# autonomousvision/unimatch

Measured on NVIDIA H100. Metric: image-pairs/sec @480x832 gmflow-scale2-refine6; EPE vs reference, higher is better.
Workload: dtype fp32

## Files before the change

### unimatch_b200/csrc/um_attention_tc.cu

```cuda
#include <math_constants.h>

#include "um_common.cuh"
#include "um_tc.cuh"

namespace um {

using namespace tc;

namespace {

constexpr int BM = 128, BN = 64;
constexpr int NTHREADS = 288;
constexpr int PRODUCER = 8;
constexpr uint32_t Q_BYTES = 4 * 16384;
constexpr uint32_t KV_STAGE_BYTES = 4 * 8192;
constexpr uint32_t OFF_Q = 0;
constexpr uint32_t OFF_K = OFF_Q + Q_BYTES;
constexpr uint32_t OFF_V = OFF_K + 2 * KV_STAGE_BYTES;
constexpr uint32_t OFF_X = OFF_V + 2 * KV_STAGE_BYTES;
constexpr uint32_t OFF_BAR = OFF_X + 1024;
constexpr uint32_t OFF_KREG = OFF_BAR + 256;
constexpr int MAX_LP = 2048;
constexpr uint32_t SMEM_BYTES = OFF_KREG + MAX_LP;
constexpr float SQRT_C = 11.313708498984761f;
constexpr float EXP_SCALE = 1.4426950408889634f / 11.313708498984761f;
constexpr float LAZY_THRESH = 8.0f / EXP_SCALE;

struct TcParams {
  float* out; long long ldo;
  int n_streams, kv_shift, lp;
  Geom g;
  const float* values; int vdim, value_mode, post_op;
  float* dbg;
  __half* out_split; long long split_plane;
};

__device__ __forceinline__ uint32_t pack_h2(__half a, __half b) {
  return (uint32_t)__half_as_ushort(a) | ((uint32_t)__half_as_ushort(b) << 16);
}

template <bool HAS_V>
__global__ void __launch_bounds__(NTHREADS, 1)
attn_tc_kernel(const __grid_constant__ CUtensorMap map_q, const __grid_constant__ CUtensorMap map_k,
               const __grid_constant__ CUtensorMap map_v, TcParams p) {
  extern __shared__ __align__(1024) uint8_t smem[];
  uint64_t* bars = reinterpret_cast<uint64_t*>(smem + OFF_BAR);
  uint64_t* q_full = bars + 0;
  uint64_t* k_full = bars + 1;
  uint64_t* k_empty = bars + 3;
  uint64_t* v_full = bars + 5;
  uint64_t* v_empty = bars + 7;
  int8_t* kreg = reinterpret_cast<int8_t*>(smem + OFF_KREG);

  const Geom g = p.g;
  const int warp = threadIdx.x >> 5, lane = threadIdx.x & 31;
  const int m0 = blockIdx.x * BM, win = blockIdx.y, n = blockIdx.z;
  const int nk = (n + p.kv_shift) % p.n_streams;
  const int nwin = g.nwin, lp = p.lp;
  const int T = (g.lw + BN - 1) / BN;
  const int planes = p.n_streams * nwin * lp;

  if (threadIdx.x == 0) {
    mbar_init(q_full, 1);
    for (int i = 0; i < 2; ++i) {
      mbar_init(k_full + i, 1); mbar_init(k_empty + i, 8);
      mbar_init(v_full + i, 1); mbar_init(v_empty + i, 8);
    }
    fence_barrier_init();
  }
  if (warp == PRODUCER && lane == 0) { tma_prefetch_desc(&map_q); tma_prefetch_desc(&map_k); tma_prefetch_desc(&map_v); }
  bool masked = false;
  if (g.mask_mode == UM_MASK_SWIN) {
    const int wy = win / g.kw, wx = win - wy * g.kw;
    masked = (g.sh > 0 && wy == g.kh - 1) || (g.sw > 0 && wx == g.kw - 1);
    if (masked)
      for (int t = threadIdx.x; t < g.lw; t += NTHREADS) {
        int yr, xr;
        window_token(g, win, t, &yr, &xr);
        kreg[t] = (int8_t)shift_region(g, yr, xr);
      }
  }
  __syncthreads();

  if (warp == PRODUCER) {
    const int qrow = (n * nwin + win) * lp + m0;
    if (elect_one()) {
      mbar_arrive_expect_tx(q_full, Q_BYTES);
#pragma unroll
      for (int part = 0; part < 2; ++part)
#pragma unroll
        for (int half = 0; half < 2; ++half)
          tma_load_2d(smem + OFF_Q + (part * 2 + half) * 16384, &map_q, q_full, half * 64, part * planes + qrow);
    }
    __syncwarp();
    const int krow = (nk * nwin + win) * lp;
    auto load_tile = [&](int j, const CUtensorMap* map, uint32_t off, uint64_t* full, uint64_t* empty) {
      const int s = j & 1;
      mbar_wait_inline(empty + s, ((j >> 1) & 1) ^ 1);
      if (elect_one()) {
        mbar_arrive_expect_tx(full + s, KV_STAGE_BYTES);
#pragma unroll
        for (int part = 0; part < 2; ++part)
#pragma unroll
          for (int half = 0; half < 2; ++half)
            tma_load_2d(smem + off + s * KV_STAGE_BYTES + (part * 2 + half) * 8192, map, full + s, half * 64,
                        part * planes + krow + j * BN);
      }
      __syncwarp();
    };
    load_tile(0, &map_k, OFF_K, k_full, k_empty);
    for (int j = 0; j < T; ++j) {
      if (j + 1 < T) load_tile(j + 1, &map_k, OFF_K, k_full, k_empty);
      if (HAS_V) load_tile(j, &map_v, OFF_V, v_full, v_empty);
    }
    return;
  }

  const int cw = warp;
  const int wg = cw >> 2;
  const int fr = wg * 64 + (cw & 3) * 16 + (lane >> 2);
  const int fc = 2 * (lane & 3);
  int rq[2] = {0, 0}, tok[2];
  bool row_valid[2];
#pragma unroll
  for (int h = 0; h < 2; ++h) {
    const int tq = m0 + fr + 8 * h;
    row_valid[h] = tq < g.lw;
    int yr = 0, xr = 0;
    tok[h] = row_valid[h] ? window_token(g, win, tq, &yr, &xr) : -1;
    if (masked) rq[h] = shift_region(g, yr, xr);
  }
  float m_run[2] = {-CUDART_INF_F, -CUDART_INF_F}, l_run[2] = {0.f, 0.f};
  const uint32_t q_base = smem_u32(smem + OFF_Q) + wg * 8192;
  auto consumers_sync = [&]() { asm volatile("bar.sync 1, 256;" ::: "memory"); };

  auto compute_s = [&](int j, float (&sv)[32]) {
    const int s = j & 1;
    mbar_wait_inline(k_full + s, (j >> 1) & 1);
    const uint32_t k_base = smem_u32(smem + OFF_K + s * KV_STAGE_BYTES);
    const int qa[3] = {1, 0, 0}, kb[3] = {0, 1, 0};
    fence_acc(sv);
    wgmma_fence();
#pragma unroll
    for (int c = 0; c < 3; ++c)
#pragma unroll
      for (int half = 0; half < 2; ++half)
#pragma unroll
        for (int ks = 0; ks < 4; ++ks)
          wgmma_ss<BN>(sv, desc_kmajor(q_base + (qa[c] * 2 + half) * 16384 + ks * 32),
                       desc_kmajor(k_base + (kb[c] * 2 + half) * 8192 + ks * 32), (c | half | ks) != 0);
    wgmma_commit();
    wgmma_wait<0>();
    fence_acc(sv);
    __syncwarp();
    if (lane == 0) mbar_arrive(k_empty + s);
  };
  mbar_wait_inline(q_full, 0);

  if (!HAS_V) {
    float* vals = reinterpret_cast<float*>(smem + OFF_X);
    const int et = threadIdx.x;
    const long long L = (long long)g.h * g.w;
    float a0[2] = {0.f, 0.f}, a1[2] = {0.f, 0.f};
    for (int j = 0; j < T; ++j) {
      const int s = j & 1;
      const int n0 = j * BN;
      if (et < BN) {
        float v0 = 0.f, v1 = 0.f;
        const int t = n0 + et;
        if (t < g.lw) {
          const int ktok = window_token(g, win, t);
          if (p.value_mode == UM_VALUE_TENSOR) {
            const float* vp = p.values + ((long long)nk * L + ktok) * p.vdim;
            v0 = __ldg(vp); v1 = (p.vdim > 1) ? __ldg(vp + 1) : 0.f;
          } else {
            const int ky = ktok / g.w;
            v0 = (float)(ktok - ky * g.w); v1 = (float)ky;
          }
        }
        vals[(s * BN + et) * 2] = v0; vals[(s * BN + et) * 2 + 1] = v1;
      }
      float sv[32];
      compute_s(j, sv);
      consumers_sync();
      const float2* vv = reinterpret_cast<const float2*>(vals + s * BN * 2);
#pragma unroll
      for (int h = 0; h < 2; ++h) {
        float mx = -CUDART_INF_F;
#pragma unroll
        for (int jj = 0; jj < 8; ++jj)
#pragma unroll
          for (int e = 0; e < 2; ++e) {
            float& x = sv[4 * jj + 2 * h + e];
            if (n0 + 8 * jj + fc + e >= g.lw) x = -CUDART_INF_F;
            mx = fmaxf(mx, x);
          }
        mx = fmaxf(mx, __shfl_xor_sync(0xffffffffu, mx, 1));
        mx = fmaxf(mx, __shfl_xor_sync(0xffffffffu, mx, 2));
        const float m_new = fmaxf(m_run[h], mx);
        const float alpha = exp2f((m_run[h] - m_new) * EXP_SCALE);
        m_run[h] = m_new;
        const float mscaled = m_new * EXP_SCALE;
        float sum = 0.f, b0 = 0.f, b1 = 0.f;
#pragma unroll
        for (int jj = 0; jj < 8; ++jj)
#pragma unroll
          for (int e = 0; e < 2; ++e) {
            const float pe = ex2_approx(fmaf(sv[4 * jj + 2 * h + e], EXP_SCALE, -mscaled));
            const float2 kv = vv[8 * jj + fc + e];
            sum += pe;
            b0 = fmaf(pe, kv.x, b0);
            b1 = fmaf(pe, kv.y, b1);
          }
        l_run[h] = l_run[h] * alpha + sum;
        a0[h] = a0[h] * alpha + b0;
        a1[h] = a1[h] * alpha + b1;
      }
    }
#pragma unroll
    for (int h = 0; h < 2; ++h) {
#pragma unroll
      for (int o = 1; o <= 2; o <<= 1) {
        l_run[h] += __shfl_xor_sync(0xffffffffu, l_run[h], o);
        a0[h] += __shfl_xor_sync(0xffffffffu, a0[h], o);
        a1[h] += __shfl_xor_sync(0xffffffffu, a1[h], o);
      }
      if (row_valid[h] && (lane & 3) == 0) {
        float r0 = a0[h] / l_run[h], r1 = a1[h] / l_run[h];
        const int oy = tok[h] / g.w, ox = tok[h] - oy * g.w;
        if (p.post_op == UM_POST_MINUS_OWN) { r0 -= (float)ox; r1 -= (float)oy; }
        else if (p.post_op == UM_POST_OWN_MINUS) { r0 = (float)ox - r0; }
        float* dst = p.out + ((long long)n * L + tok[h]) * p.vdim;
        dst[0] = r0;
        if (p.vdim > 1) dst[1] = r1;
      }
    }
    return;
  }

  float o[64];
#pragma unroll
  for (int i = 0; i < 64; ++i) o[i] = 0.f;
  const bool dump = p.dbg && blockIdx.x == 0 && blockIdx.y == 0 && blockIdx.z == 0;
  for (int j = 0; j < T; ++j) {
    const int s = j & 1;
    const int n0 = j * BN;
    float sv[32];
    compute_s(j, sv);
    if (dump && j == 0)
#pragma unroll
      for (int i = 0; i < 32; ++i) p.dbg[(fr + 8 * ((i >> 1) & 1)) * BN + 8 * (i >> 2) + fc + (i & 1)] = sv[i];
    uint32_t ph[16], pl[16];
#pragma unroll
    for (int h = 0; h < 2; ++h) {
#pragma unroll
      for (int jj = 0; jj < 8; ++jj)
#pragma unroll
        for (int e = 0; e < 2; ++e) {
          const int col = n0 + 8 * jj + fc + e;
          float& x = sv[4 * jj + 2 * h + e];
          if (masked && kreg[col < g.lw ? col : 0] != rq[h]) x -= 100.0f * SQRT_C;
          if (col >= g.lw) x = -CUDART_INF_F;
        }
      float mx = -CUDART_INF_F;
#pragma unroll
      for (int jj = 0; jj < 8; ++jj) mx = fmaxf(mx, fmaxf(sv[4 * jj + 2 * h], sv[4 * jj + 2 * h + 1]));
      mx = fmaxf(mx, __shfl_xor_sync(0xffffffffu, mx, 1));
      mx = fmaxf(mx, __shfl_xor_sync(0xffffffffu, mx, 2));
      float alpha = 1.0f;
      if (mx > m_run[h] + LAZY_THRESH) {
        alpha = exp2f((m_run[h] - mx) * EXP_SCALE);
        m_run[h] = mx;
#pragma unroll
        for (int jj = 0; jj < 16; ++jj) { o[4 * jj + 2 * h] *= alpha; o[4 * jj + 2 * h + 1] *= alpha; }
      }
      const float mscaled = m_run[h] * EXP_SCALE;
      float sum = 0.f;
#pragma unroll
      for (int jj = 0; jj < 8; ++jj) {
        const float p0 = ex2_approx(fmaf(sv[4 * jj + 2 * h], EXP_SCALE, -mscaled));
        const float p1 = ex2_approx(fmaf(sv[4 * jj + 2 * h + 1], EXP_SCALE, -mscaled));
        sum += p0 + p1;
        split_f16x2(p0, p1, &ph[2 * jj + h], &pl[2 * jj + h]);
      }
      l_run[h] = l_run[h] * alpha + sum;
    }
    mbar_wait_inline(v_full + s, (j >> 1) & 1);
    const uint32_t v_base = smem_u32(smem + OFF_V + s * KV_STAGE_BYTES);
    fence_acc(o);
    wgmma_fence();
#pragma unroll
    for (int c = 0; c < 3; ++c)
#pragma unroll
      for (int ks = 0; ks < 4; ++ks) {
        const uint32_t* pp = c == 0 ? pl : ph;
        const uint32_t a[4] = {pp[4 * ks], pp[4 * ks + 1], pp[4 * ks + 2], pp[4 * ks + 3]};
        wgmma_rs_n128_tb(o, a, desc_mnmajor(v_base + (c == 1 ? 16384 : 0) + ks * 2048, 8192), true);
      }
    wgmma_commit();
    wgmma_wait<0>();
    fence_acc(o);
    __syncwarp();
    if (lane == 0) mbar_arrive(v_empty + s);
  }

  float inv[2];
#pragma unroll
  for (int h = 0; h < 2; ++h) {
    float l = l_run[h];
    l += __shfl_xor_sync(0xffffffffu, l, 1);
    l += __shfl_xor_sync(0xffffffffu, l, 2);
    inv[h] = 1.0f / l;
  }
  consumers_sync();
  float* osm = reinterpret_cast<float*>(smem + OFF_Q);
#pragma unroll
  for (int jj = 0; jj < 16; ++jj)
#pragma unroll
    for (int h = 0; h < 2; ++h) {
      const int row = fr + 8 * h, col = 8 * jj + fc;
      if (dump) { p.dbg[BM * BN + row * 128 + col] = o[4 * jj + 2 * h]; p.dbg[BM * BN + row * 128 + col + 1] = o[4 * jj + 2 * h + 1]; }
      *reinterpret_cast<float2*>(osm + row * 128 + (((col >> 2) ^ (row & 31)) << 2) + (col & 3)) =
          make_float2(o[4 * jj + 2 * h] * inv[h], o[4 * jj + 2 * h + 1] * inv[h]);
    }
  consumers_sync();
  float* obase = p.out + (long long)n * g.h * g.w * p.ldo;
  for (int row = cw * 16; row < cw * 16 + 16; ++row) {
    const int tq = m0 + row;
    if (tq >= g.lw) break;
    const int tk = window_token(g, win, tq);
    const float4 v = *reinterpret_cast<const float4*>(osm + row * 128 + ((lane ^ (row & 31)) << 2));
    if (p.out) *reinterpret_cast<float4*>(obase + (long long)tk * p.ldo + lane * 4) = v;
    if (p.out_split) {
      uint32_t h0, h1, l0, l1;
      split_f16x2(v.x, v.y, &h0, &l0);
      split_f16x2(v.z, v.w, &h1, &l1);
      __half* d = p.out_split + ((long long)n * g.h * g.w + tk) * 128 + lane * 4;
      *reinterpret_cast<uint2*>(d) = make_uint2(h0, h1);
      *reinterpret_cast<uint2*>(d + p.split_plane) = make_uint2(l0, l1);
    }
  }
}

struct SplitParams {
  const float* src[3]; long long ld[3];
  __half* dst[3];
  int n_streams, lp;
  Geom g;
};

__global__ void __launch_bounds__(256) split_windows_kernel(SplitParams p) {
  const Geom g = p.g;
  const int lane = threadIdx.x & 31;
  const int t = blockIdx.x * 8 + (threadIdx.x >> 5);
  const int win = blockIdx.y, n = blockIdx.z;
  if (t >= p.lp) return;
  const long long planes = (long long)p.n_streams * g.nwin * p.lp;
  const long long row = ((long long)n * g.nwin + win) * p.lp + t;
  const int tok = (t < g.lw) ? window_token(g, win, t) : -1;
#pragma unroll
  for (int a = 0; a < 3; ++a) {
    if (!p.src[a]) continue;
    float4 x = make_float4(0.f, 0.f, 0.f, 0.f);
    if (tok >= 0) x = __ldg(reinterpret_cast<const float4*>(p.src[a] + ((long long)n * g.h * g.w + tok) * p.ld[a]) + lane);
    __half h[4], l[4];
    split_f16(x.x, &h[0], &l[0]); split_f16(x.y, &h[1], &l[1]);
    split_f16(x.z, &h[2], &l[2]); split_f16(x.w, &h[3], &l[3]);
    uint2 hv = make_uint2(pack_h2(h[0], h[1]), pack_h2(h[2], h[3]));
    uint2 lv = make_uint2(pack_h2(l[0], l[1]), pack_h2(l[2], l[3]));
    reinterpret_cast<uint2*>(p.dst[a] + row * 128)[lane] = hv;
    reinterpret_cast<uint2*>(p.dst[a] + (planes + row) * 128)[lane] = lv;
  }
}

}

PFN_encodeTiled get_encode_tiled() {
  static PFN_encodeTiled fn = nullptr;
  if (!fn) {
    void* sym = nullptr;
    cudaDriverEntryPointQueryResult qres;
    if (cudaGetDriverEntryPoint("cuTensorMapEncodeTiled", &sym, cudaEnableDefault, &qres) == cudaSuccess &&
        qres == cudaDriverEntryPointSuccess)
      fn = reinterpret_cast<PFN_encodeTiled>(sym);
  }
  return fn;
}

int make_map_2d_f16(CUtensorMap* map, const void* base, uint64_t rows, uint64_t cols, uint32_t box_rows) {
  PFN_encodeTiled enc = get_encode_tiled();
  if (!enc) { set_error("cuTensorMapEncodeTiled unavailable (no CUDA driver?)"); return UM_ECUDA; }
  cuuint64_t dims[2] = {cols, rows};
  cuuint64_t strides[1] = {cols * 2};
  cuuint32_t box[2] = {64, box_rows};
  cuuint32_t estr[2] = {1, 1};
  CUresult r = enc(map, CU_TENSOR_MAP_DATA_TYPE_FLOAT16, 2, const_cast<void*>(base), dims, strides, box, estr,
                   CU_TENSOR_MAP_INTERLEAVE_NONE, CU_TENSOR_MAP_SWIZZLE_128B, CU_TENSOR_MAP_L2_PROMOTION_L2_128B,
                   CU_TENSOR_MAP_FLOAT_OOB_FILL_NONE);
  if (r != CUDA_SUCCESS) { set_error("cuTensorMapEncodeTiled failed (%d)", (int)r); return UM_ECUDA; }
  return UM_OK;
}

static inline int padded_lw(int lw) { return (lw + 127) / 128 * 128; }

bool expectation_tc_supported(const Geom& g, int value_mode) {
  return g.kh == 1 && g.kw == 1 && g.lw >= BM && g.mask_mode == UM_MASK_NONE && g.sh == 0 && g.sw == 0 &&
         (value_mode == UM_VALUE_TENSOR || value_mode == UM_VALUE_COORDS);
}

size_t expectation_tc_workspace_bytes(const Geom& g, int n_total) {
  return (size_t)2 * 2 * n_total * g.nwin * padded_lw(g.lw) * 128 * sizeof(__half);
}

bool attention_tc_supported(const Geom& g) {
  return g.lw >= BM && padded_lw(g.lw) <= MAX_LP && (g.mask_mode == UM_MASK_NONE || g.mask_mode == UM_MASK_SWIN);
}

size_t attention_tc_workspace_bytes(const Geom& g, int n_streams) {
  return (size_t)3 * 2 * n_streams * g.nwin * padded_lw(g.lw) * 128 * sizeof(__half);
}

int split_windows_launch(const float* q, const float* k, const float* v, long long ldq, long long ldk, long long ldv,
                         __half* wq, __half* wk, __half* wv, int n_streams, const Geom& g, cudaStream_t st, const char* what) {
  SplitParams sp{};
  sp.src[0] = q; sp.src[1] = k; sp.src[2] = v;
  sp.ld[0] = ldq; sp.ld[1] = ldk; sp.ld[2] = ldv;
  sp.dst[0] = wq; sp.dst[1] = wk; sp.dst[2] = wv;
  sp.n_streams = n_streams; sp.lp = padded_lw(g.lw); sp.g = g;
  split_windows_kernel<<<dim3((sp.lp + 7) / 8, g.nwin, n_streams), 256, 0, st>>>(sp);
  return check_launch(what);
}


int attention_planes_launch(const __half* wq, const __half* wk, const __half* wv, float* out, long long ldo, __half* out_split,
                               long long split_plane, int n_streams, int kv_shift, const Geom& g, float* dbg, cudaStream_t st) {
  const int lp = padded_lw(g.lw);
  int rc;
  CUtensorMap mq, mk, mv;
  const uint64_t rows = (uint64_t)2 * n_streams * g.nwin * lp;
  if ((rc = make_map_2d_f16(&mq, wq, rows, 128, BM))) return rc;
  if ((rc = make_map_2d_f16(&mk, wk, rows, 128, BN))) return rc;
  if ((rc = make_map_2d_f16(&mv, wv, rows, 128, BN))) return rc;
  static PerDeviceBytes configured;
  if ((rc = ensure_smem(configured, attn_tc_kernel<true>, SMEM_BYTES, "attn_tc"))) return rc;
  TcParams p{};
  p.out = out; p.ldo = ldo; p.n_streams = n_streams; p.kv_shift = kv_shift; p.lp = lp; p.g = g; p.dbg = dbg;
  p.out_split = out_split; p.split_plane = split_plane;
  const int qtiles = (g.lw + BM - 1) / BM;
  attn_tc_kernel<true><<<dim3(qtiles, g.nwin, n_streams), NTHREADS, SMEM_BYTES, st>>>(mq, mk, mv, p);
  return check_launch("um_window_attention(wgmma)");
}

int window_attention_tc(const float* q, const float* k, const float* v, float* out, int n_streams, int kv_shift,
                        long long ldq, long long ldk, long long ldv, long long ldo, const Geom& g, void* workspace,
                        float* dbg, cudaStream_t st, int* rows_done) {
  const int lp = padded_lw(g.lw);
  const size_t plane_elems = (size_t)2 * n_streams * g.nwin * lp * 128;
  __half* wq = reinterpret_cast<__half*>(workspace);
  __half* wk = wq + plane_elems;
  __half* wv = wk + plane_elems;
  int rc = split_windows_launch(q, k, v, ldq, ldk, ldv, wq, wk, wv, n_streams, g, st, "um_window_attention(split)");
  if (rc) return rc;
  *rows_done = g.lw;
  return attention_planes_launch(wq, wk, wv, out, ldo, nullptr, 0, n_streams, kv_shift, g, dbg, st);
}

int softmax_expectation_tc(const float* q, const float* k, const float* values, float* out, int n_streams, int n_total,
                           int kv_shift, long long ldq, long long ldk, int vdim, int value_mode, int post_op,
                           const Geom& g, void* workspace, cudaStream_t st) {
  const int lp = padded_lw(g.lw);
  const size_t plane_elems = (size_t)2 * n_total * g.nwin * lp * 128;
  __half* wq = reinterpret_cast<__half*>(workspace);
  __half* wk = wq + plane_elems;
  int rc = split_windows_launch(q, k, nullptr, ldq, ldk, 0, wq, wk, nullptr, n_total, g, st, "um_softmax_expectation(split)");
  if (rc) return rc;
  CUtensorMap mq, mk;
  const uint64_t rows = (uint64_t)2 * n_total * g.nwin * lp;
  if ((rc = make_map_2d_f16(&mq, wq, rows, 128, BM))) return rc;
  if ((rc = make_map_2d_f16(&mk, wk, rows, 128, BN))) return rc;
  static PerDeviceBytes configured;
  if ((rc = ensure_smem(configured, attn_tc_kernel<false>, SMEM_BYTES, "expect_tc"))) return rc;
  TcParams p{};
  p.out = out; p.ldo = vdim; p.n_streams = n_total; p.kv_shift = kv_shift; p.lp = lp; p.g = g; p.dbg = nullptr;
  p.values = values; p.vdim = vdim; p.value_mode = value_mode; p.post_op = post_op;
  const int qtiles = (g.lw + BM - 1) / BM;
  attn_tc_kernel<false><<<dim3(qtiles, g.nwin, n_streams), NTHREADS, SMEM_BYTES, st>>>(mq, mk, mk, p);
  return check_launch("um_softmax_expectation(wgmma)");
}

}
```

### unimatch_b200/csrc/um_ffn_tc.cu

```cuda
#include "um_common.cuh"
#include "um_tc.cuh"

namespace um {

using namespace tc;

namespace {

constexpr int NTHREADS = 288;
constexpr int PRODUCER = 8;
constexpr int HC = 64;
constexpr uint32_t X_BYTES = 4 * 32768;
constexpr uint32_t SLOT_BYTES = 16384;
constexpr int NSLOT = 5;
constexpr uint32_t OFF_RING = X_BYTES;
constexpr uint32_t OFF_BAR = OFF_RING + NSLOT * SLOT_BYTES;
constexpr uint32_t SMEM_BYTES = OFF_BAR + 256;
static_assert(SMEM_BYTES <= 232448, "shared memory budget");

struct FfnParams {
  int nchunk, hidden;
  const float* residual; long long ld_res;
  const float* gamma; const float* beta;
  float* out_f32; long long ld_f32;
  __half* out_split; long long split_plane;
};

__global__ void __launch_bounds__(NTHREADS, 1)
ffn_tc_kernel(const __grid_constant__ CUtensorMap map_x0, const __grid_constant__ CUtensorMap map_x1,
              const __grid_constant__ CUtensorMap map_w1, const __grid_constant__ CUtensorMap map_w2, FfnParams p) {
  extern __shared__ __align__(1024) uint8_t smem[];
  uint64_t* bars = reinterpret_cast<uint64_t*>(smem + OFF_BAR);
  uint64_t* x_full = bars;
  uint64_t* full = bars + 1;
  uint64_t* empty = bars + 1 + NSLOT;
  const int warp = threadIdx.x >> 5, lane = threadIdx.x & 31;
  const int tile = blockIdx.x;

  if (threadIdx.x == 0) {
    mbar_init(x_full, 1);
    for (int i = 0; i < NSLOT; ++i) { mbar_init(full + i, 1); mbar_init(empty + i, 8); }
    fence_barrier_init();
  }
  if (warp == PRODUCER && lane == 0) {
    tma_prefetch_desc(&map_x0); tma_prefetch_desc(&map_x1); tma_prefetch_desc(&map_w1); tma_prefetch_desc(&map_w2);
  }
  __syncthreads();

  if (warp == PRODUCER) {
    if (elect_one()) {
      mbar_arrive_expect_tx(x_full, X_BYTES);
#pragma unroll
      for (int kc = 0; kc < 4; ++kc)
#pragma unroll
        for (int part = 0; part < 2; ++part)
          tma_load_4d(smem + (kc * 2 + part) * 16384, kc < 2 ? &map_x0 : &map_x1, x_full, (kc & 1) * 64, 0, tile * 8, part);
    }
    __syncwarp();
    int it = 0;
    for (int c = 0; c < p.nchunk; ++c)
      for (int q = 0; q < 6; ++q, ++it) {
        const int s = it % NSLOT;
        mbar_wait_inline(empty + s, ((it / NSLOT) & 1) ^ 1);
        uint8_t* slot = smem + OFF_RING + s * SLOT_BYTES;
        if (elect_one()) {
          mbar_arrive_expect_tx(full + s, SLOT_BYTES);
#pragma unroll
          for (int part = 0; part < 2; ++part) {
            if (q < 4) tma_load_2d(slot + part * 8192, &map_w1, full + s, q * 64, part * p.hidden + c * HC);
            else tma_load_2d(slot + part * 8192, &map_w2, full + s, c * HC, part * 128 + (q - 4) * 64);
          }
        }
        __syncwarp();
      }
    return;
  }

  const int wg = warp >> 2;
  const int fr = wg * 64 + (warp & 3) * 16 + (lane >> 2);
  const int fc = 2 * (lane & 3);
  const uint32_t x_base = smem_u32(smem) + wg * 8192;
  const int pa[3] = {1, 0, 0}, pb[3] = {0, 1, 0};
  float o[64];
#pragma unroll
  for (int i = 0; i < 64; ++i) o[i] = 0.f;
  mbar_wait_inline(x_full, 0);
  int it = 0;
  for (int c = 0; c < p.nchunk; ++c) {
    float h[32];
    int sl[4];
#pragma unroll
    for (int q = 0; q < 4; ++q) {
      sl[q] = (it + q) % NSLOT;
      mbar_wait_inline(full + sl[q], ((it + q) / NSLOT) & 1);
    }
    fence_acc(h);
    wgmma_fence();
#pragma unroll
    for (int q = 0; q < 4; ++q) {
      const uint32_t sb = smem_u32(smem + OFF_RING + sl[q] * SLOT_BYTES);
#pragma unroll
      for (int cc = 0; cc < 3; ++cc)
#pragma unroll
        for (int ks = 0; ks < 4; ++ks)
          wgmma_ss<64>(h, desc_kmajor(x_base + (q * 2 + pa[cc]) * 16384 + ks * 32), desc_kmajor(sb + pb[cc] * 8192 + ks * 32),
                       (q | cc | ks) != 0);
    }
    wgmma_commit();
    wgmma_wait<0>();
    fence_acc(h);
    __syncwarp();
    if (lane == 0)
#pragma unroll
      for (int q = 0; q < 4; ++q) mbar_arrive(empty + sl[q]);
    it += 4;
    uint32_t ph[16], pl[16];
#pragma unroll
    for (int jj = 0; jj < 8; ++jj)
#pragma unroll
      for (int hh = 0; hh < 2; ++hh)
        split_f16x2(act_gelu(h[4 * jj + 2 * hh]), act_gelu(h[4 * jj + 2 * hh + 1]), &ph[2 * jj + hh], &pl[2 * jj + hh]);
#pragma unroll
    for (int q = 0; q < 2; ++q) {
      sl[q] = (it + q) % NSLOT;
      mbar_wait_inline(full + sl[q], ((it + q) / NSLOT) & 1);
    }
    fence_acc(o);
    wgmma_fence();
#pragma unroll
    for (int q = 0; q < 2; ++q) {
      const uint32_t sb = smem_u32(smem + OFF_RING + sl[q] * SLOT_BYTES);
      float (&oq)[32] = *reinterpret_cast<float (*)[32]>(o + 32 * q);
#pragma unroll
      for (int cc = 0; cc < 3; ++cc)
#pragma unroll
        for (int ks = 0; ks < 4; ++ks) {
          const uint32_t* pp = cc == 0 ? pl : ph;
          const uint32_t a[4] = {pp[4 * ks], pp[4 * ks + 1], pp[4 * ks + 2], pp[4 * ks + 3]};
          wgmma_rs_n64(oq, a, desc_kmajor(sb + (cc == 1 ? 8192 : 0) + ks * 32), true);
        }
    }
    wgmma_commit();
    wgmma_wait<0>();
    fence_acc(o);
    __syncwarp();
    if (lane == 0) { mbar_arrive(empty + sl[0]); mbar_arrive(empty + sl[1]); }
    it += 2;
  }

#pragma unroll
  for (int hh = 0; hh < 2; ++hh) {
    const long long row = (long long)tile * 128 + fr + 8 * hh;
    float sum = 0.f;
#pragma unroll
    for (int jj = 0; jj < 16; ++jj) sum += o[4 * jj + 2 * hh] + o[4 * jj + 2 * hh + 1];
    sum += __shfl_xor_sync(0xffffffffu, sum, 1);
    sum += __shfl_xor_sync(0xffffffffu, sum, 2);
    const float mean = sum * (1.0f / 128.0f);
    float sq = 0.f;
#pragma unroll
    for (int jj = 0; jj < 16; ++jj) {
      const float d0 = o[4 * jj + 2 * hh] - mean, d1 = o[4 * jj + 2 * hh + 1] - mean;
      sq = fmaf(d0, d0, fmaf(d1, d1, sq));
    }
    sq += __shfl_xor_sync(0xffffffffu, sq, 1);
    sq += __shfl_xor_sync(0xffffffffu, sq, 2);
    const float rstd = rsqrtf(sq * (1.0f / 128.0f) + 1e-5f);
#pragma unroll
    for (int jj = 0; jj < 16; ++jj) {
      const int col = 8 * jj + fc;
      float y0 = (o[4 * jj + 2 * hh] - mean) * rstd * __ldg(p.gamma + col) + __ldg(p.beta + col);
      float y1 = (o[4 * jj + 2 * hh + 1] - mean) * rstd * __ldg(p.gamma + col + 1) + __ldg(p.beta + col + 1);
      if (p.residual) {
        const float2 r = __ldg(reinterpret_cast<const float2*>(p.residual + row * p.ld_res + col));
        y0 += r.x; y1 += r.y;
      }
      if (p.out_f32) *reinterpret_cast<float2*>(p.out_f32 + row * p.ld_f32 + col) = make_float2(y0, y1);
      if (p.out_split) {
        uint32_t hi, lo;
        split_f16x2(y0, y1, &hi, &lo);
        *reinterpret_cast<uint32_t*>(p.out_split + row * 128 + col) = hi;
        *reinterpret_cast<uint32_t*>(p.out_split + p.split_plane + row * 128 + col) = lo;
      }
    }
  }
}

}
}

extern "C" {

int um_ffn_tc(const um_ffn_desc* d, void* stream) {
  UM_REQUIRE(d && d->src[0] && d->src[1] && d->w1 && d->w2 && d->gamma && d->beta, "um_ffn_tc: null descriptor / operand");
  UM_REQUIRE(d->rows > 0 && d->rows % 256 == 0, "um_ffn_tc: rows must be a positive multiple of 256 (pairs of 128-row tiles)");
  UM_REQUIRE(d->hidden >= 128 && d->hidden % 128 == 0, "um_ffn_tc: hidden must be a multiple of 128");
  UM_REQUIRE(d->out_f32 || d->out_split, "um_ffn_tc: no output");
  UM_REQUIRE(d->src_plane_stride >= d->rows * 128 && d->src_plane_stride % 8 == 0,
             "um_ffn_tc: source plane stride must cover rows * 128 halves (multiple of 8)");
  if (d->residual)
    UM_REQUIRE(d->ld_res % 4 == 0 && d->ld_res >= 128 && (reinterpret_cast<uintptr_t>(d->residual) & 15) == 0,
               "um_ffn_tc: residual rows must be 16-byte aligned");
  if (d->out_f32)
    UM_REQUIRE(d->ld_f32 % 4 == 0 && d->ld_f32 >= 128 && (reinterpret_cast<uintptr_t>(d->out_f32) & 15) == 0,
               "um_ffn_tc: fp32 output rows must be 16-byte aligned");
  if (d->out_split)
    UM_REQUIRE(d->split_plane_stride >= d->rows * 128 && d->split_plane_stride % 8 == 0 &&
                   (reinterpret_cast<uintptr_t>(d->out_split) & 15) == 0,
               "um_ffn_tc: output plane stride must cover rows * 128 halves (multiple of 8), 16-byte aligned planes");
  using namespace um;
  const uint64_t gh = (uint64_t)d->rows / 16;
  CUtensorMap mx0, mx1, mw1, mw2;
  int rc;
  if ((rc = make_map_4d_f16(&mx0, d->src[0], 128, 16, gh, 2, 1, (uint64_t)d->src_plane_stride))) return rc;
  if ((rc = make_map_4d_f16(&mx1, d->src[1], 128, 16, gh, 2, 1, (uint64_t)d->src_plane_stride))) return rc;
  if ((rc = make_map_2d_f16(&mw1, d->w1, 2ull * d->hidden, 256, 64))) return rc;
  if ((rc = make_map_2d_f16(&mw2, d->w2, 2ull * 128, (uint64_t)d->hidden, 64))) return rc;
  FfnParams p{};
  p.nchunk = d->hidden / HC; p.hidden = d->hidden;
  p.residual = d->residual; p.ld_res = d->ld_res; p.gamma = d->gamma; p.beta = d->beta;
  p.out_f32 = d->out_f32; p.ld_f32 = d->ld_f32;
  p.out_split = reinterpret_cast<__half*>(d->out_split); p.split_plane = d->split_plane_stride;
  static PerDeviceBytes configured;
  if ((rc = ensure_smem(configured, ffn_tc_kernel, SMEM_BYTES, "ffn_tc"))) return rc;
  ffn_tc_kernel<<<(unsigned)(d->rows / 128), NTHREADS, SMEM_BYTES, (cudaStream_t)stream>>>(mx0, mx1, mw1, mw2, p);
  return check_launch("um_ffn_tc");
}

}
```

Before: 65.08.

## Software-pipeline QK and PV wgmma in attention and FFN consumer loops

Both the attention and FFN consumer loops are restructured so the next block's first GEMM (QK^T or X·W1) is issued before the current block's second GEMM (P·V or H·W2). Softmax or GELU then runs while tensor cores are busy, and wgmma_wait<1> is used to separate the two in-flight groups. Attention also skips consumer warpgroups whose query rows lie past the window length, lowering the empty-barrier reader count to match. FFN adds a fourth warpgroup so it can reallocate registers with setmaxnreg (producer down, consumers up) and grows the ring to 6 slots. The risks are register pressure from holding sv/h alongside o and the P fragments, and possible barrier-phase mistakes.

```diff
diff --git a/unimatch_b200/csrc/um_attention_tc.cu b/unimatch_b200/csrc/um_attention_tc.cu
--- a/unimatch_b200/csrc/um_attention_tc.cu
+++ b/unimatch_b200/csrc/um_attention_tc.cu
@@ -61,10 +61,11 @@
   const int planes = p.n_streams * nwin * lp;
 
   if (threadIdx.x == 0) {
+    const uint32_t readers = (HAS_V && g.lw - m0 <= 64) ? 4 : 8;
     mbar_init(q_full, 1);
     for (int i = 0; i < 2; ++i) {
-      mbar_init(k_full + i, 1); mbar_init(k_empty + i, 8);
-      mbar_init(v_full + i, 1); mbar_init(v_empty + i, 8);
+      mbar_init(k_full + i, 1); mbar_init(k_empty + i, readers);
+      mbar_init(v_full + i, 1); mbar_init(v_empty + i, readers);
     }
     fence_barrier_init();
   }
@@ -242,66 +243,128 @@
 #pragma unroll
   for (int i = 0; i < 64; ++i) o[i] = 0.f;
   const bool dump = p.dbg && blockIdx.x == 0 && blockIdx.y == 0 && blockIdx.z == 0;
-  for (int j = 0; j < T; ++j) {
-    const int s = j & 1;
-    const int n0 = j * BN;
+  const bool active = m0 + wg * 64 < g.lw;
+  if (active) {
     float sv[32];
-    compute_s(j, sv);
-    if (dump && j == 0)
+    uint32_t ph[16], pl[16];
+    float alpha[2] = {1.0f, 1.0f};
+    bool rescale[2] = {false, false};
+    auto issue_s = [&](int j) {
+      const int s = j & 1;
+      mbar_wait_inline(k_full + s, (j >> 1) & 1);
+      const uint32_t k_base = smem_u32(smem + OFF_K + s * KV_STAGE_BYTES);
+      const int qa[3] = {1, 0, 0}, kb[3] = {0, 1, 0};
+      fence_acc(sv);
+      wgmma_fence();
+#pragma unroll
+      for (int c = 0; c < 3; ++c)
+#pragma unroll
+        for (int half = 0; half < 2; ++half)
+#pragma unroll
+          for (int ks = 0; ks < 4; ++ks)
+            wgmma_ss<BN>(sv, desc_kmajor(q_base + (qa[c] * 2 + half) * 16384 + ks * 32),
+                         desc_kmajor(k_base + (kb[c] * 2 + half) * 8192 + ks * 32), (c | half | ks) != 0);
+      wgmma_commit();
+    };
+    auto release_k = [&](int j) {
+      fence_acc(sv);
+      __syncwarp();
+      if (lane == 0) mbar_arrive(k_empty + (j & 1));
+    };
+    auto softmax = [&](int j) {
+      const int n0 = j * BN;
+#pragma unroll
+      for (int h = 0; h < 2; ++h) {
+#pragma unroll
+        for (int jj = 0; jj < 8; ++jj)
+#pragma unroll
+          for (int e = 0; e < 2; ++e) {
+            const int col = n0 + 8 * jj + fc + e;
+            float& x = sv[4 * jj + 2 * h + e];
+            if (masked && kreg[col < g.lw ? col : 0] != rq[h]) x -= 100.0f * SQRT_C;
+            if (col >= g.lw) x = -CUDART_INF_F;
+          }
+        float mx = -CUDART_INF_F;
+#pragma unroll
+        for (int jj = 0; jj < 8; ++jj) mx = fmaxf(mx, fmaxf(sv[4 * jj + 2 * h], sv[4 * jj + 2 * h + 1]));
+        mx = fmaxf(mx, __shfl_xor_sync(0xffffffffu, mx, 1));
+        mx = fmaxf(mx, __shfl_xor_sync(0xffffffffu, mx, 2));
+        float a = 1.0f;
+        rescale[h] = mx > m_run[h] + LAZY_THRESH;
+        if (rescale[h]) {
+          a = exp2f((m_run[h] - mx) * EXP_SCALE);
+          m_run[h] = mx;
+        }
+        alpha[h] = a;
+        const float mscaled = m_run[h] * EXP_SCALE;
+        float sum = 0.f;
+#pragma unroll
+        for (int jj = 0; jj < 8; ++jj) {
+          const float p0 = ex2_approx(fmaf(sv[4 * jj + 2 * h], EXP_SCALE, -mscaled));
+          const float p1 = ex2_approx(fmaf(sv[4 * jj + 2 * h + 1], EXP_SCALE, -mscaled));
+          sum += p0 + p1;
+          sv[4 * jj + 2 * h] = p0;
+          sv[4 * jj + 2 * h + 1] = p1;
+        }
+        l_run[h] = l_run[h] * a + sum;
+      }
+    };
+    auto split_p = [&]() {
+#pragma unroll
+      for (int jj = 0; jj < 8; ++jj)
+#pragma unroll
+        for (int h = 0; h < 2; ++h)
+          split_f16x2(sv[4 * jj + 2 * h], sv[4 * jj + 2 * h + 1], &ph[2 * jj + h], &pl[2 * jj + h]);
+    };
+
+    auto issue_pv = [&](int j) {
+#pragma unroll
+      for (int h = 0; h < 2; ++h)
+        if (rescale[h])
+#pragma unroll
+          for (int jj = 0; jj < 16; ++jj) { o[4 * jj + 2 * h] *= alpha[h]; o[4 * jj + 2 * h + 1] *= alpha[h]; }
+      const int s = j & 1;
+      mbar_wait_inline(v_full + s, (j >> 1) & 1);
+      const uint32_t v_base = smem_u32(smem + OFF_V + s * KV_STAGE_BYTES);
+      fence_acc(o);
+      wgmma_fence();
+#pragma unroll
+      for (int c = 0; c < 3; ++c)
+#pragma unroll
+        for (int ks = 0; ks < 4; ++ks) {
+          const uint32_t* pp = c == 0 ? pl : ph;
+          const uint32_t a[4] = {pp[4 * ks], pp[4 * ks + 1], pp[4 * ks + 2], pp[4 * ks + 3]};
+          wgmma_rs_n128_tb(o, a, desc_mnmajor(v_base + (c == 1 ? 16384 : 0) + ks * 2048, 8192), true);
+        }
+      wgmma_commit();
+    };
+    auto release_v = [&](int j) {
+      fence_acc(o);
+      __syncwarp();
+      if (lane == 0) mbar_arrive(v_empty + (j & 1));
+    };
+
+    issue_s(0);
+    wgmma_wait<0>();
+    release_k(0);
+    if (dump)
 #pragma unroll
       for (int i = 0; i < 32; ++i) p.dbg[(fr + 8 * ((i >> 1) & 1)) * BN + 8 * (i >> 2) + fc + (i & 1)] = sv[i];
-    uint32_t ph[16], pl[16];
-#pragma unroll
-    for (int h = 0; h < 2; ++h) {
-#pragma unroll
-      for (int jj = 0; jj < 8; ++jj)
-#pragma unroll
-        for (int e = 0; e < 2; ++e) {
-          const int col = n0 + 8 * jj + fc + e;
-          float& x = sv[4 * jj + 2 * h + e];
-          if (masked && kreg[col < g.lw ? col : 0] != rq[h]) x -= 100.0f * SQRT_C;
-          if (col >= g.lw) x = -CUDART_INF_F;
-        }
-      float mx = -CUDART_INF_F;
-#pragma unroll
-      for (int jj = 0; jj < 8; ++jj) mx = fmaxf(mx, fmaxf(sv[4 * jj + 2 * h], sv[4 * jj + 2 * h + 1]));
-      mx = fmaxf(mx, __shfl_xor_sync(0xffffffffu, mx, 1));
-      mx = fmaxf(mx, __shfl_xor_sync(0xffffffffu, mx, 2));
-      float alpha = 1.0f;
-      if (mx > m_run[h] + LAZY_THRESH) {
-        alpha = exp2f((m_run[h] - mx) * EXP_SCALE);
-        m_run[h] = mx;
-#pragma unroll
-        for (int jj = 0; jj < 16; ++jj) { o[4 * jj + 2 * h] *= alpha; o[4 * jj + 2 * h + 1] *= alpha; }
-      }
-      const float mscaled = m_run[h] * EXP_SCALE;
-      float sum = 0.f;
-#pragma unroll
-      for (int jj = 0; jj < 8; ++jj) {
-        const float p0 = ex2_approx(fmaf(sv[4 * jj + 2 * h], EXP_SCALE, -mscaled));
-        const float p1 = ex2_approx(fmaf(sv[4 * jj + 2 * h + 1], EXP_SCALE, -mscaled));
-        sum += p0 + p1;
-        split_f16x2(p0, p1, &ph[2 * jj + h], &pl[2 * jj + h]);
-      }
-      l_run[h] = l_run[h] * alpha + sum;
-    }
-    mbar_wait_inline(v_full + s, (j >> 1) & 1);
-    const uint32_t v_base = smem_u32(smem + OFF_V + s * KV_STAGE_BYTES);
-    fence_acc(o);
-    wgmma_fence();
-#pragma unroll
-    for (int c = 0; c < 3; ++c)
-#pragma unroll
-      for (int ks = 0; ks < 4; ++ks) {
-        const uint32_t* pp = c == 0 ? pl : ph;
-        const uint32_t a[4] = {pp[4 * ks], pp[4 * ks + 1], pp[4 * ks + 2], pp[4 * ks + 3]};
-        wgmma_rs_n128_tb(o, a, desc_mnmajor(v_base + (c == 1 ? 16384 : 0) + ks * 2048, 8192), true);
-      }
-    wgmma_commit();
+    softmax(0);
+    split_p();
+    for (int j = 0; j + 1 < T; ++j) {
+      issue_s(j + 1);
+      issue_pv(j);
+      wgmma_wait<1>();
+      release_k(j + 1);
+      softmax(j + 1);
+      wgmma_wait<0>();
+      release_v(j);
+      split_p();
+    }
+    issue_pv(T - 1);
     wgmma_wait<0>();
-    fence_acc(o);
-    __syncwarp();
-    if (lane == 0) mbar_arrive(v_empty + s);
+    release_v(T - 1);
   }
 
   float inv[2];
diff --git a/unimatch_b200/csrc/um_ffn_tc.cu b/unimatch_b200/csrc/um_ffn_tc.cu
--- a/unimatch_b200/csrc/um_ffn_tc.cu
+++ b/unimatch_b200/csrc/um_ffn_tc.cu
@@ -7,12 +7,13 @@
 
 namespace {
 
-constexpr int NTHREADS = 288;
+constexpr int NTHREADS = 384;
 constexpr int PRODUCER = 8;
+constexpr int REGS_PRODUCER = 40, REGS_CONSUMER = 232;
 constexpr int HC = 64;
 constexpr uint32_t X_BYTES = 4 * 32768;
 constexpr uint32_t SLOT_BYTES = 16384;
-constexpr int NSLOT = 5;
+constexpr int NSLOT = 6;
 constexpr uint32_t OFF_RING = X_BYTES;
 constexpr uint32_t OFF_BAR = OFF_RING + NSLOT * SLOT_BYTES;
 constexpr uint32_t SMEM_BYTES = OFF_BAR + 256;
@@ -35,7 +36,6 @@
   uint64_t* full = bars + 1;
   uint64_t* empty = bars + 1 + NSLOT;
   const int warp = threadIdx.x >> 5, lane = threadIdx.x & 31;
-  const int tile = blockIdx.x;
 
   if (threadIdx.x == 0) {
     mbar_init(x_full, 1);
@@ -47,7 +47,10 @@
   }
   __syncthreads();
 
-  if (warp == PRODUCER) {
+  if (warp >= PRODUCER) {
+    setmaxnreg_dec<REGS_PRODUCER>();
+    if (warp != PRODUCER) return;
+    const int tile = blockIdx.x;
     if (elect_one()) {
       mbar_arrive_expect_tx(x_full, X_BYTES);
 #pragma unroll
@@ -76,6 +79,8 @@
     return;
   }
 
+  setmaxnreg_inc<REGS_CONSUMER>();
+  const int tile = blockIdx.x;
   const int wg = warp >> 2;
   const int fr = wg * 64 + (warp & 3) * 16 + (lane >> 2);
   const int fc = 2 * (lane & 3);
@@ -84,21 +89,23 @@
   float o[64];
 #pragma unroll
   for (int i = 0; i < 64; ++i) o[i] = 0.f;
-  mbar_wait_inline(x_full, 0);
-  int it = 0;
-  for (int c = 0; c < p.nchunk; ++c) {
-    float h[32];
-    int sl[4];
-#pragma unroll
-    for (int q = 0; q < 4; ++q) {
-      sl[q] = (it + q) % NSLOT;
-      mbar_wait_inline(full + sl[q], ((it + q) / NSLOT) & 1);
-    }
+  float h[32];
+  uint32_t ph[16], pl[16];
+  auto item_wait = [&](int i) { mbar_wait_inline(full + i % NSLOT, (i / NSLOT) & 1); };
+  auto item_smem = [&](int i) { return smem_u32(smem + OFF_RING + (i % NSLOT) * SLOT_BYTES); };
+  auto release = [&](int i0, int n) {
+    __syncwarp();
+    if (lane == 0)
+      for (int i = i0; i < i0 + n; ++i) mbar_arrive(empty + i % NSLOT);
+  };
+  auto issue_h = [&](int c) {
+#pragma unroll
+    for (int q = 0; q < 4; ++q) item_wait(6 * c + q);
     fence_acc(h);
     wgmma_fence();
 #pragma unroll
     for (int q = 0; q < 4; ++q) {
-      const uint32_t sb = smem_u32(smem + OFF_RING + sl[q] * SLOT_BYTES);
+      const uint32_t sb = item_smem(6 * c + q);
 #pragma unroll
       for (int cc = 0; cc < 3; ++cc)
 #pragma unroll
@@ -107,29 +114,27 @@
                        (q | cc | ks) != 0);
     }
     wgmma_commit();
-    wgmma_wait<0>();
-    fence_acc(h);
-    __syncwarp();
-    if (lane == 0)
-#pragma unroll
-      for (int q = 0; q < 4; ++q) mbar_arrive(empty + sl[q]);
-    it += 4;
-    uint32_t ph[16], pl[16];
+  };
+  auto gelu_h = [&]() {
+#pragma unroll
+    for (int i = 0; i < 32; ++i) h[i] = act_gelu(h[i]);
+  };
+  auto split_h = [&]() {
 #pragma unroll
     for (int jj = 0; jj < 8; ++jj)
 #pragma unroll
       for (int hh = 0; hh < 2; ++hh)
-        split_f16x2(act_gelu(h[4 * jj + 2 * hh]), act_gelu(h[4 * jj + 2 * hh + 1]), &ph[2 * jj + hh], &pl[2 * jj + hh]);
-#pragma unroll
-    for (int q = 0; q < 2; ++q) {
-      sl[q] = (it + q) % NSLOT;
-      mbar_wait_inline(full + sl[q], ((it + q) / NSLOT) & 1);
-    }
+        split_f16x2(h[4 * jj + 2 * hh], h[4 * jj + 2 * hh + 1], &ph[2 * jj + hh], &pl[2 * jj + hh]);
+  };
+
+  auto issue_o = [&](int c) {
+    item_wait(6 * c + 4);
+    item_wait(6 * c + 5);
     fence_acc(o);
     wgmma_fence();
 #pragma unroll
     for (int q = 0; q < 2; ++q) {
-      const uint32_t sb = smem_u32(smem + OFF_RING + sl[q] * SLOT_BYTES);
+      const uint32_t sb = item_smem(6 * c + 4 + q);
       float (&oq)[32] = *reinterpret_cast<float (*)[32]>(o + 32 * q);
 #pragma unroll
       for (int cc = 0; cc < 3; ++cc)
@@ -141,12 +146,31 @@
         }
     }
     wgmma_commit();
+  };
+
+  mbar_wait_inline(x_full, 0);
+  issue_h(0);
+  wgmma_wait<0>();
+  fence_acc(h);
+  release(0, 4);
+  gelu_h();
+  split_h();
+  for (int c = 0; c + 1 < p.nchunk; ++c) {
+    issue_h(c + 1);
+    issue_o(c);
+    wgmma_wait<1>();
+    fence_acc(h);
+    release(6 * (c + 1), 4);
+    gelu_h();
     wgmma_wait<0>();
     fence_acc(o);
-    __syncwarp();
-    if (lane == 0) { mbar_arrive(empty + sl[0]); mbar_arrive(empty + sl[1]); }
-    it += 2;
-  }
+    release(6 * c + 4, 2);
+    split_h();
+  }
+  issue_o(p.nchunk - 1);
+  wgmma_wait<0>();
+  fence_acc(o);
+  release(6 * (p.nchunk - 1) + 4, 2);
 
 #pragma unroll
   for (int hh = 0; hh < 2; ++hh) {
```

Result: faster. 66.33 (median of 6 runs) (+1.9%).

## Ping-pong schedule two consumer warpgroups for attention MMA and softmax

Applied to the files above, without the earlier changes.

Restructures the attention main loop so each consumer warpgroup issues the P·V MMA of the previous tile together with the Q·K MMA of the next tile in one turn. Named barriers alternate turns between the two warpgroups, so one warpgroup's tensor-core work overlaps the other's softmax. This targets tensor-core idle time during the exponent and rescale math, at the cost of extra barrier synchronisation and a more fragile turn-passing protocol.

```diff
diff --git a/unimatch_b200/csrc/um_attention_tc.cu b/unimatch_b200/csrc/um_attention_tc.cu
--- a/unimatch_b200/csrc/um_attention_tc.cu
+++ b/unimatch_b200/csrc/um_attention_tc.cu
@@ -242,15 +242,60 @@
 #pragma unroll
   for (int i = 0; i < 64; ++i) o[i] = 0.f;
   const bool dump = p.dbg && blockIdx.x == 0 && blockIdx.y == 0 && blockIdx.z == 0;
-  for (int j = 0; j < T; ++j) {
+  auto wait_turn = [&]() { asm volatile("bar.sync %0, 256;" ::"r"(2 + wg) : "memory"); };
+  auto pass_turn = [&]() { asm volatile("bar.arrive %0, 256;" ::"r"(3 - wg) : "memory"); };
+  uint32_t ph[16], pl[16];
+  float sv[32];
+  auto issue_pv = [&](int j) {
+    const int sp = j & 1;
+    mbar_wait_inline(v_full + sp, (j >> 1) & 1);
+    const uint32_t v_base = smem_u32(smem + OFF_V + sp * KV_STAGE_BYTES);
+#pragma unroll
+    for (int c = 0; c < 3; ++c)
+#pragma unroll
+      for (int ks = 0; ks < 4; ++ks) {
+        const uint32_t* pp = c == 0 ? pl : ph;
+        const uint32_t a[4] = {pp[4 * ks], pp[4 * ks + 1], pp[4 * ks + 2], pp[4 * ks + 3]};
+        wgmma_rs_n128_tb(o, a, desc_mnmajor(v_base + (c == 1 ? 16384 : 0) + ks * 2048, 8192), true);
+      }
+  };
+  auto issue_s = [&](int j) {
     const int s = j & 1;
+    mbar_wait_inline(k_full + s, (j >> 1) & 1);
+    const uint32_t k_base = smem_u32(smem + OFF_K + s * KV_STAGE_BYTES);
+    const int qa[3] = {1, 0, 0}, kb[3] = {0, 1, 0};
+#pragma unroll
+    for (int c = 0; c < 3; ++c)
+#pragma unroll
+      for (int half = 0; half < 2; ++half)
+#pragma unroll
+        for (int ks = 0; ks < 4; ++ks)
+          wgmma_ss<BN>(sv, desc_kmajor(q_base + (qa[c] * 2 + half) * 16384 + ks * 32),
+                       desc_kmajor(k_base + (kb[c] * 2 + half) * 8192 + ks * 32), (c | half | ks) != 0);
+  };
+  auto mma_turn = [&](int j_pv, int j_s, bool pass) {
+    wait_turn();
+    fence_acc(o);
+    fence_acc(sv);
+    wgmma_fence();
+    if (j_pv >= 0) issue_pv(j_pv);
+    if (j_s >= 0) issue_s(j_s);
+    wgmma_commit();
+    if (pass) pass_turn();
+    wgmma_wait<0>();
+    fence_acc(o);
+    fence_acc(sv);
+    __syncwarp();
+    if (lane == 0) {
+      if (j_s >= 0) mbar_arrive(k_empty + (j_s & 1));
+      if (j_pv >= 0) mbar_arrive(v_empty + (j_pv & 1));
+    }
+  };
+  auto softmax = [&](int j) {
     const int n0 = j * BN;
-    float sv[32];
-    compute_s(j, sv);
     if (dump && j == 0)
 #pragma unroll
       for (int i = 0; i < 32; ++i) p.dbg[(fr + 8 * ((i >> 1) & 1)) * BN + 8 * (i >> 2) + fc + (i & 1)] = sv[i];
-    uint32_t ph[16], pl[16];
 #pragma unroll
     for (int h = 0; h < 2; ++h) {
 #pragma unroll
@@ -285,24 +330,15 @@
       }
       l_run[h] = l_run[h] * alpha + sum;
     }
-    mbar_wait_inline(v_full + s, (j >> 1) & 1);
-    const uint32_t v_base = smem_u32(smem + OFF_V + s * KV_STAGE_BYTES);
-    fence_acc(o);
-    wgmma_fence();
-#pragma unroll
-    for (int c = 0; c < 3; ++c)
-#pragma unroll
-      for (int ks = 0; ks < 4; ++ks) {
-        const uint32_t* pp = c == 0 ? pl : ph;
-        const uint32_t a[4] = {pp[4 * ks], pp[4 * ks + 1], pp[4 * ks + 2], pp[4 * ks + 3]};
-        wgmma_rs_n128_tb(o, a, desc_mnmajor(v_base + (c == 1 ? 16384 : 0) + ks * 2048, 8192), true);
-      }
-    wgmma_commit();
-    wgmma_wait<0>();
-    fence_acc(o);
-    __syncwarp();
-    if (lane == 0) mbar_arrive(v_empty + s);
-  }
+  };
+  if (wg == 1) pass_turn();
+  mma_turn(-1, 0, true);
+  softmax(0);
+  for (int j = 1; j < T; ++j) {
+    mma_turn(j - 1, j, true);
+    softmax(j);
+  }
+  mma_turn(T - 1, -1, wg == 0);
 
   float inv[2];
 #pragma unroll
```

Measured after the change: 81.67 before, 83.09 after, median of 6. 1.7% higher.
